# Anttwo/SuGaR

Hardware: AMD Instinct MI355X
Metric: train_step_images_per_sec (higher is better)
Workload: dtype f32; 1 GPU; metric: 1000000 Gaussians @ 1920x1080, SH degree 3, 3DGS train step (raster fwd -> 0.8 L1 + 0.2 DSSIM -> bwd -> Adam, 59 floats/Gaussian), 8 orbit cameras cycled; parallelism=view-sharded dp1, single process, no collective

## Files before the change

### include/sugar_raster.h

```cpp
#ifndef SUGAR_RASTER_H_INCLUDED
#define SUGAR_RASTER_H_INCLUDED

#include <stddef.h>
#include <stdint.h>

#ifdef __cplusplus
extern "C" {
#endif

#define SGR_ABI_VERSION 4

#define SGR_E_INVALID (-1)
#define SGR_E_HIP (-2)
#define SGR_E_ALLOC (-3)

typedef char* (*sgr_alloc_fn)(void* user, size_t bytes);

int sgr_abi_version(void);
const char* sgr_last_error(void);

int64_t sgr_forward(sgr_alloc_fn geom_alloc, void* geom_user,
                    sgr_alloc_fn binning_alloc, void* binning_user,
                    sgr_alloc_fn img_alloc, void* img_user,
                    int P, int D, int M,
// ... 78 lines not shown
                       char* geom_buffer, char* binning_buffer, char* img_buffer,
                       const float* dL_dpix,
                       float* dL_dmean2D, float* dL_dconic, float* dL_dopacity, float* dL_dcolor,
                       float* dL_dmean3D, float* dL_dcov3D, float* dL_dsh, float* dL_dscale, float* dL_drot,
                       int debug, void* stream);

typedef struct sgr_backward_opts {
    float* max_radii2D;
    float* grad_accum;
    float* denom;
    float* campos_row;
    int flags;
} sgr_backward_opts;
#define SGR_BWD_EXACT_ALPHA 2
#define SGR_BWD_TILE_ORDER_READY 1
int sgr_backward_ex(int phase, int P, int D, int M, int64_t R,
                    const float* background, int width, int height,
                    const float* means3D, const float* shs, const float* colors_precomp,
                    const float* scales, float scale_modifier, const float* rotations,
                    const float* cov3D_precomp, const float* viewmatrix, const float* projmatrix,
                    const float* cam_pos, float tan_fovx, float tan_fovy, const int* radii,
                    char* geom_buffer, char* binning_buffer, char* img_buffer,
                    const float* dL_dpix,
                    float* dL_dmean2D, float* dL_dconic, float* dL_dopacity, float* dL_dcolor,
                    float* dL_dmean3D, float* dL_dcov3D, float* dL_dsh, float* dL_dscale, float* dL_drot,
                    int debug, void* stream, const sgr_backward_opts* opts);

int sgr_sh_grad_from_views(int P, int n_views, int D, int M, const float* means3D, const float* campos_all,
                           const float* dcolor_all, int64_t view_stride, float* dL_dsh, void* stream);

// ... 3 lines not shown
                           float lr_rest, float beta1, float beta2, float eps, int step, float grad_scale, void* stream);

int sgr_sh_adam_from_views_ex(int P, int n_views, int D, int M, const float* means3D, const float* campos_all,
                              const float* dcolor_all, int64_t view_stride, float* sh_params, float* exp_avg, float* exp_avg_sq,
                              float lr_dc, float lr_rest, float beta1, float beta2, float eps, int step, float grad_scale,
                              float* dmean_extra, void* stream);

int sgr_mark_visible(int P, const float* means3D, const float* viewmatrix, const float* projmatrix,
                     uint8_t* present, void* stream);

size_t sgr_geom_bytes(int P);
size_t sgr_img_bytes(int width, int height);
size_t sgr_binning_bytes(int64_t R, int width, int height);

size_t sgr_geom_rec_offset(int P);
size_t sgr_img_final_T_offset(int width, int height);
size_t sgr_img_n_contrib_offset(int width, int height);
size_t sgr_img_tile_start_offset(int width, int height);
size_t sgr_img_tile_maxc_offset(int width, int height);
size_t sgr_img_tile_walked_offset(int width, int height);
size_t sgr_img_header_offset(int width, int height);
size_t sgr_binning_point_list_offset(int64_t R);

#define SGR_N_STAGES 15
void sgr_profile_enable(int stage_mask);
int sgr_profile_read(double* ms_sum, int64_t* count, int n_stages);


int sgr_dist2(int P, const float* points, float* meanDists, void* stream);
int sgr_knn(int N, const float* query, int M, const float* ref, int K, float* dists, int64_t* idx, void* stream);
// ... 62 lines not shown
    int64_t view_stride;
    const float* all_campos;
    float grad_scale;
    int step;
    int64_t g_begin, g_end;
    int64_t f_begin, f_end;
} sgr_train_exchange;
typedef struct sgr_trainer sgr_trainer;
sgr_trainer* sgr_trainer_create(const sgr_train_config* cfg);
void sgr_trainer_destroy(sgr_trainer* t);
int sgr_trainer_set_binning(sgr_trainer* t, char* binning, size_t bytes, int64_t capacity);
int sgr_trainer_step(sgr_trainer* t, const sgr_train_view* view, int phases, const sgr_train_exchange* ex, void* stream);
int sgr_trainer_set_exchange_chunks(sgr_trainer* t, int n);
int sgr_trainer_forward_valid(sgr_trainer* t, uint32_t* header_out);
const char* sgr_trainer_last_error(void);
int sgr_rccl_unique_id(char* out128);
int sgr_trainer_comm_init(sgr_trainer* t, const char* id128, int world, int rank, float* recv, size_t recv_bytes);
int sgr_trainer_comm_destroy(sgr_trainer* t);
int sgr_trainer_comm_abort(sgr_trainer* t);
int sgr_trainer_step_exchange(sgr_trainer* t, const sgr_train_view* view, int step, void* stream);
double sgr_trainer_last_exchange_wait_ms(sgr_trainer* t);
size_t sgr_bin2_bytes(int P, int width, int height);

int sgr_scaled_rotation_forward(int P, const float* quaternions, const float* scaling, int inverse_scales, float* out,
                                void* stream);
int sgr_scaled_rotation_backward(int P, const float* quaternions, const float* scaling, int inverse_scales,
                                 const float* dL_dout, float* dL_dquaternions, float* dL_dscaling, void* stream);

int sgr_pack_gaussians(int P, const float* centers, const float* inv_scaled_rot, const float* strengths, float* packed,
                       void* stream);
// ... 119 lines not shown
```

### sugar_amd/_lib.py

```python
from __future__ import annotations

import ctypes as C
import os

_HERE = os.path.dirname(os.path.abspath(__file__))
LIB_PATH = os.environ.get("SGR_LIB_PATH") or os.path.join(_HERE, "libsugar_raster.so")

ALLOC_FN = C.CFUNCTYPE(C.c_void_p, C.c_void_p, C.c_size_t)

_vp, _i, _f, _i64, _sz = C.c_void_p, C.c_int, C.c_float, C.c_int64, C.c_size_t
SIGNATURES = {
    "sgr_abi_version": (_i, []),
    "sgr_last_error": (C.c_char_p, []),
    "sgr_set_deep_min": (None, [_i]),
    "sgr_get_deep_min": (_i, []),
    "sgr_set_exact_alpha": (None, [_i]),
    "sgr_get_exact_alpha": (_i, []),
    "sgr_forward": (_i64, [ALLOC_FN, _vp, ALLOC_FN, _vp, ALLOC_FN, _vp, _i, _i, _i, _vp, _i, _i, _vp, _vp, _vp, _vp,
                           _vp, _f, _vp, _vp, _vp, _vp, _vp, _f, _f, _i, _vp, _vp, _i, _vp]),
    "sgr_forward_ex": (_i64, [ALLOC_FN, _vp, ALLOC_FN, _vp, ALLOC_FN, _vp, _i, _i, _i, _vp, _i, _i, _vp, _vp, _vp, _vp,
                              _vp, _f, _vp, _vp, _vp, _vp, _vp, _f, _f, _i, _vp, _vp, _i, _vp, _vp]),
    "sgr_backward": (_i, [_i, _i, _i, _i64, _vp, _i, _i, _vp, _vp, _vp, _vp, _f, _vp, _vp, _vp, _vp, _vp, _f, _f, _vp,
                          _vp, _vp, _vp, _vp, _vp, _vp, _vp, _vp, _vp, _vp, _vp, _vp, _vp, _i, _vp]),
    "sgr_backward_phase": (_i, [_i, _i, _i, _i, _i64, _vp, _i, _i, _vp, _vp, _vp, _vp, _f, _vp, _vp, _vp, _vp, _vp, _f, _f, _vp,
                                _vp, _vp, _vp, _vp, _vp, _vp, _vp, _vp, _vp, _vp, _vp, _vp, _vp, _i, _vp]),
    "sgr_backward_ex": (_i, [_i, _i, _i, _i, _i64, _vp, _i, _i, _vp, _vp, _vp, _vp, _f, _vp, _vp, _vp, _vp, _vp, _f, _f, _vp,
                             _vp, _vp, _vp, _vp, _vp, _vp, _vp, _vp, _vp, _vp, _vp, _vp, _vp, _i, _vp, _vp]),
    "sgr_mark_visible": (_i, [_i, _vp, _vp, _vp, _vp, _vp]),
    "sgr_trainer_create": (_vp, [_vp]),
    "sgr_trainer_destroy": (None, [_vp]),
    "sgr_trainer_set_binning": (_i, [_vp, _vp, _sz, _i64]),
    "sgr_trainer_step": (_i, [_vp, _vp, _i, _vp, _vp]),
    "sgr_trainer_forward_valid": (_i, [_vp, _vp]),
    "sgr_trainer_last_error": (C.c_char_p, []),
    "sgr_rccl_unique_id": (_i, [_vp]),
    "sgr_trainer_comm_init": (_i, [_vp, _vp, _i, _i, _vp, _sz]),
    "sgr_trainer_comm_destroy": (_i, [_vp]),
    "sgr_trainer_comm_abort": (_i, [_vp]),
    "sgr_trainer_step_exchange": (_i, [_vp, _vp, _i, _vp]),
    "sgr_trainer_set_exchange_chunks": (_i, [_vp, _i]),
    "sgr_trainer_last_exchange_wait_ms": (C.c_double, [_vp]),
    "sgr_bin2_bytes": (_sz, [_i, _i, _i]),
    "sgr_sh_grad_from_views": (_i, [_i, _i, _i, _i, _vp, _vp, _vp, _i64, _vp, _vp]),
    "sgr_sh_adam_from_views": (_i, [_i, _i, _i, _i, _vp, _vp, _vp, _i64, _vp, _vp, _vp, _f, _f, _f, _f, _f, _i, _f, _vp]),
    "sgr_sh_adam_from_views_ex": (_i, [_i, _i, _i, _i, _vp, _vp, _vp, _i64, _vp, _vp, _vp, _f, _f, _f, _f, _f, _i, _f, _vp, _vp]),
    "sgr_geom_bytes": (_sz, [_i]),
    "sgr_img_bytes": (_sz, [_i, _i]),
    "sgr_binning_bytes": (_sz, [_i64, _i, _i]),
    "sgr_geom_rec_offset": (_sz, [_i]),
    "sgr_img_final_T_offset": (_sz, [_i, _i]),
    "sgr_img_n_contrib_offset": (_sz, [_i, _i]),
    "sgr_img_tile_start_offset": (_sz, [_i, _i]),
    "sgr_img_tile_maxc_offset": (_sz, [_i, _i]),
    "sgr_img_tile_walked_offset": (_sz, [_i, _i]),
    "sgr_img_header_offset": (_sz, [_i, _i]),
    "sgr_binning_point_list_offset": (_sz, [_i64]),
    "sgr_profile_enable": (None, [_i]),
    "sgr_profile_read": (_i, [_vp, _vp, _i]),
    "sgr_l1_ssim_scratch_bytes": (_sz, [_i, _i, _i]),
    "sgr_l1_ssim_forward": (_i, [_i, _i, _i, _vp, _vp, _f, _vp, _vp, _vp]),
    "sgr_l1_ssim_backward": (_i, [_i, _i, _i, _vp, _vp, _f, _vp, _vp, _vp, _vp]),
    "sgr_l1_ssim_backward_ex": (_i, [_i, _i, _i, _vp, _vp, _f, _vp, _vp, _vp, _vp, _vp]),
    "sgr_adam_step": (_i, [C.c_longlong, _vp, _vp, _vp, _vp, _i, _vp, _vp, _vp, _vp, _vp, _vp, _f, _f, _f, _i, _f, _vp]),
    "sgr_adam_step_multi": (_i, [_i, _vp, _vp, _vp, _vp, _vp, _vp, _vp, _vp, _vp, _vp, _vp]),
# ... 84 lines not shown
                ("max_radii2D", _vp), ("grad_accum", _vp), ("denom", _vp)]


class TrainView(C.Structure):
    _fields_ = [("viewmatrix", _vp), ("projmatrix", _vp), ("campos", _vp), ("tan_fovx", _f), ("tan_fovy", _f), ("gt_image", _vp),
                ("tile_need", _vp), ("tile_need_out", _vp), ("hint_margin", _f), ("chunk_grid", C.c_uint32),
                ("tile_order", _vp), ("tile_order_out", _vp), ("flags", C.c_uint32)]


class TrainExchange(C.Structure):
    _fields_ = [("n_views", _i), ("all_colors", _vp), ("view_stride", _i64), ("all_campos", _vp), ("grad_scale", _f), ("step", _i),
                ("g_begin", _i64), ("g_end", _i64), ("f_begin", _i64), ("f_end", _i64)]


SGR_FLAG_RAW_PARAMS, SGR_FLAG_SINGLE_LEVEL_BINNING, SGR_FLAG_SPECULATIVE = 1, 2, 8
SGR_BWD_TILE_ORDER_READY = 1
HDR_R, HDR_HINT_MISS, HDR_L1_OVERFLOW = 0, 3, 6

_lib = None


def load() -> C.CDLL:
    global _lib
    if _lib is not None:
        return _lib
    if not os.path.exists(LIB_PATH):
        raise ImportError(
            f"{LIB_PATH} not found: the gfx950 HIP rasterizer is not built. Run `python -m sugar_amd.build` "
            "(or __graft_entry__.build()). There is no CPU fallback.")
    lib = C.CDLL(LIB_PATH)
    for name, (res, args) in SIGNATURES.items():
# ... 15 lines not shown
```

### sugar_amd/csrc/capi.hip

```cpp
#include "../../include/sugar_raster.h"
#include "sgr_common.h"
#include "tile_order.h"

#include <cstdlib>
#include <mutex>
#include <string>
#include <vector>

namespace {

thread_local std::string g_err;

int fail(int code, const std::string& msg)
{
    g_err = msg;
    return code;
}

#define HIP_TRY(expr)                                                                                   \
    do {                                                                                                \
        hipError_t e_ = (expr);                                                                         \
        if (e_ != hipSuccess)                                                                           \
            return fail(SGR_E_HIP, std::string(#expr) + ": " + hipGetErrorString(e_));                  \
    } while (0)
// ... 92 lines not shown

extern "C" {

int sgr_abi_version(void) { return SGR_ABI_VERSION; }
void sgr_set_deep_min(int entries) { g_deep_min = entries > 0 ? entries : 0; }
int sgr_get_deep_min(void) { return (int)sgr_deep_min(); }
void sgr_set_exact_alpha(int on) { g_exact_alpha = on ? 1 : 0; }
int sgr_get_exact_alpha(void) { return sgr_exact_alpha(); }

const char* sgr_last_error(void) { return g_err.c_str(); }

size_t sgr_geom_bytes(int P) { return sgr_geom_total(P); }
size_t sgr_img_bytes(int width, int height) { return sgr_img_layout(width, height).total; }
size_t sgr_binning_bytes(int64_t R, int width, int height) { return sgr_bin_layout(R, sgr_img_layout(width, height).T).total; }
size_t sgr_geom_rec_offset(int) { return 0; }
size_t sgr_img_final_T_offset(int w, int h) { return sgr_img_layout(w, h).final_T; }
size_t sgr_img_n_contrib_offset(int w, int h) { return sgr_img_layout(w, h).n_contrib; }
size_t sgr_img_tile_start_offset(int w, int h) { return sgr_img_layout(w, h).tile_start; }
size_t sgr_img_tile_maxc_offset(int w, int h) { return sgr_img_layout(w, h).tile_maxc; }
size_t sgr_img_tile_walked_offset(int w, int h) { return sgr_img_layout(w, h).tile_walked; }
size_t sgr_img_header_offset(int w, int h) { return sgr_img_layout(w, h).header; }
size_t sgr_binning_point_list_offset(int64_t R) { return sgr_bin_layout(R, 0).point_list; }

void sgr_profile_enable(int stage_mask) { g_prof.mask = (unsigned)stage_mask; }

int sgr_profile_read(double* ms_sum, int64_t* count, int n_stages)
{
    std::lock_guard<std::mutex> lk(g_prof_mu);
    for (int i = 0; i < n_stages; i++) { ms_sum[i] = 0.0; count[i] = 0; }
    for (auto& r : g_prof.recs) {
// ... 284 lines not shown
    job->T = IL.T;
    job->list_cap = (uint32_t)(R > 0xFFFFFFFFll ? 0xFFFFFFFFll : R);
    job->tile_maxc = reinterpret_cast<const uint32_t*>(img_buffer + IL.tile_maxc);
    job->tile_walked = opts->tile_need_out ? reinterpret_cast<const uint32_t*>(img_buffer + IL.tile_walked) : nullptr;
    job->header = reinterpret_cast<const uint32_t*>(img_buffer + IL.header);
    job->order = reinterpret_cast<uint32_t*>(img_buffer + IL.tile_cursor);
    job->order_copy = opts->tile_order_out;
    job->need_out = opts->tile_need_out;
    job->header_host = hh_dev;
    job->margin = opts->hint_margin > 0.f ? opts->hint_margin : 0.25f;
    job->gx = IL.gx;
    job->gy = IL.gy;
    return 0;
}

static int backward_impl(int phase, int P, int D, int M, int64_t R, const float* background, int width, int height,
                         const float* means3D, const float* shs, const float* colors_precomp, const float* scales,
                         float scale_modifier, const float* rotations, const float* cov3D_precomp, const float* viewmatrix,
                         const float* projmatrix, const float* cam_pos, float tan_fovx, float tan_fovy, char* geom_buffer,
                         char* binning_buffer, char* img_buffer, const float* dL_dpix, float* dL_dmean2D, float* dL_dconic,
                         float* dL_dopacity, float* dL_dcolor, float* dL_dmean3D, float* dL_dcov3D, float* dL_dsh,
                         float* dL_dscale, float* dL_drot, int debug, void* stream, const sgr_backward_opts* opts = nullptr)
{
    hipStream_t s = (hipStream_t)stream;
    const int raw_params = (phase & SGR_MODE_RAW_PARAMS) ? 1 : 0;
    const int sh_dir_elsewhere = (phase & SGR_MODE_SH_DIR_ELSEWHERE) ? 1 : 0;
    phase &= 3;
    if (phase < 0 || phase > 2) return fail(SGR_E_INVALID, "phase must be 0, 1 or 2");
    if (P <= 0 || width <= 0 || height <= 0) return fail(SGR_E_INVALID, "P, width and height must be positive");
    if (!geom_buffer || !binning_buffer || !img_buffer || !dL_dpix) return fail(SGR_E_INVALID, "null scratch / dL_dpix");
    if (!dL_dopacity || !dL_dcolor || !dL_dmean3D) return fail(SGR_E_INVALID, "null gradient output");
    if (cov3D_precomp && !dL_dcov3D) return fail(SGR_E_INVALID, "dL_dcov3D required with cov3D_precomp");
    const bool use_sh = shs && !colors_precomp;
    const bool compact = use_sh && !dL_dsh;
    if (!cov3D_precomp && (!dL_dscale || !dL_drot)) return fail(SGR_E_INVALID, "dL_dscale/dL_drot required");
    if (phase != 0 && !compact) return fail(SGR_E_INVALID, "the two-phase backward is for the compact SH mode");

    const ImgLayout IL = sgr_img_layout(width, height);
    const BinLayout BL = sgr_bin_layout(R, IL.T);
    const GeomRec* rec = reinterpret_cast<const GeomRec*>(geom_buffer);
    const float* final_T = reinterpret_cast<const float*>(img_buffer + IL.final_T);
    const uint32_t* n_contrib = reinterpret_cast<const uint32_t*>(img_buffer + IL.n_contrib);
    const uint32_t* tile_start = reinterpret_cast<const uint32_t*>(img_buffer + IL.tile_start);
    const uint32_t* blk_nb = reinterpret_cast<const uint32_t*>(img_buffer + IL.blk_nb);
    const uint32_t* point_list = reinterpret_cast<const uint32_t*>(binning_buffer + BL.point_list);

    float* acc = reinterpret_cast<float*>(geom_buffer + sgr_geom_acc_offset(P));
    if (phase != 2) {
        { SgrStageTimer t(s, SGR_STAGE_FILL); HIP_TRY(hipMemsetAsync(acc, 0, (size_t)P * SGR_ACC_STRIDE * 4, s)); }
        if (R > 0) {
            SgrStageTimer t(s, SGR_STAGE_BLEND_BWD);
            sgr_launch_blend_bwd(width, height, IL.gx, IL.gy, tile_start, point_list, binning_buffer, blk_nb, rec, background, final_T,
                                 n_contrib, dL_dpix, acc, reinterpret_cast<const uint32_t*>(img_buffer + IL.tile_maxc),
                                 reinterpret_cast<const uint32_t*>(img_buffer + IL.header), (uint32_t)(R > 0xFFFFFFFFll ? 0xFFFFFFFFll : R),
                                 reinterpret_cast<uint32_t*>(img_buffer + IL.tile_cursor),
                                 (opts && (opts->flags & SGR_BWD_TILE_ORDER_READY)) ? 1 : 0, s,
                                 (sgr_exact_alpha() || (opts && (opts->flags & SGR_BWD_EXACT_ALPHA))) ? 1 : 0);
        }
        STAGE_CHECK("blend_bwd");
        if (phase == 1) {
            { SgrStageTimer t(s, SGR_STAGE_MASKED_COLORS); sgr_launch_masked_colors(P, rec, acc, dL_dcolor, cam_pos, opts ? opts->campos_row : nullptr, s); }
            STAGE_CHECK("masked_colors");
            return 0;
        }
    }
    PreprocessBwdArgs pb;
    pb.P = P; pb.D = D; pb.M = use_sh ? M : 0;
    pb.means3D = means3D; pb.shs = use_sh ? shs : nullptr;
    pb.scales = cov3D_precomp ? nullptr : scales; pb.rotations = cov3D_precomp ? nullptr : rotations;
    pb.scale_modifier = scale_modifier; pb.cov3D_precomp = cov3D_precomp;
    pb.viewmatrix = viewmatrix; pb.projmatrix = projmatrix; pb.cam_pos = cam_pos;
    pb.W = width; pb.H = height; pb.tan_fovx = tan_fovx; pb.tan_fovy = tan_fovy;
    pb.focal_y = height / (2.0f * tan_fovy);
    pb.focal_x = width / (2.0f * tan_fovx);
    pb.rec = rec;
    pb.raw_params = raw_params && !cov3D_precomp;
    pb.sh_dir_elsewhere = sh_dir_elsewhere && use_sh && !dL_dsh;
    pb.acc = acc;
    pb.header = reinterpret_cast<const uint32_t*>(img_buffer + IL.header);
    pb.list_cap = (uint32_t)(R > 0xFFFFFFFFll ? 0xFFFFFFFFll : R);
    pb.campos_row = (opts && compact && phase == 0) ? opts->campos_row : nullptr;
    pb.dens_max_radii = opts ? opts->max_radii2D : nullptr;
    pb.dens_accum = opts ? opts->grad_accum : nullptr;
    pb.dens_denom = opts ? opts->denom : nullptr;
    pb.dL_dmean2D = dL_dmean2D; pb.dL_dconic = dL_dconic; pb.dL_dopacity = dL_dopacity;
    pb.dL_dcolor = phase == 2 ? nullptr : dL_dcolor;
    pb.dL_dmean3D = dL_dmean3D; pb.dL_dcov3D = dL_dcov3D; pb.dL_dsh = use_sh ? dL_dsh : nullptr;
    pb.dL_dscale = cov3D_precomp ? nullptr : dL_dscale; pb.dL_drot = cov3D_precomp ? nullptr : dL_drot;
    { SgrStageTimer t(s, SGR_STAGE_PREPROCESS_BWD); sgr_launch_preprocess_bwd(pb, s); }
    STAGE_CHECK("preprocess_bwd");
    return 0;
}

// ... 104 lines not shown
```

### sugar_amd/csrc/preprocess.hip

```cpp
#include "../../include/sugar_raster.h"
#include "sgr_common.h"

namespace {

__device__ __constant__ const float SH_C0 = 0.28209479177387814f;
__device__ __constant__ const float SH_C1 = 0.4886025119029199f;
__device__ __constant__ const float SH_C2[5] = {1.0925484305920792f, -1.0925484305920792f, 0.31539156525252005f,
                                                 -1.0925484305920792f, 0.5462742152960396f};
__device__ __constant__ const float SH_C3[7] = {-0.5900435899266435f, 2.890611442640554f, -0.4570457994644658f,
                                                 0.3731763325901154f, -0.4570457994644658f, 1.445305721320277f,
                                                 -0.5900435899266435f};

__device__ __forceinline__ float fmin_(float a, float b) { return a < b ? a : b; }
__device__ __forceinline__ float fmax_(float a, float b) { return a > b ? a : b; }

__device__ __forceinline__ int f2i_sat(float v)
{
    if (v != v) return 0;
    if (v >= 2147483648.0f) return 2147483647;
    if (v <= -2147483648.0f) return (-2147483647 - 1);
    return (int)v;
}

__device__ __forceinline__ float ndc2pix(float v, int S)
// ... 381 lines not shown
    uint32_t kmin = key, kmax = key == 0xFFFFFFFFu ? 0u : key;
    for (int o = 32; o > 0; o >>= 1) {
        kmin = min(kmin, (uint32_t)__shfl_xor((int)kmin, o));
        kmax = max(kmax, (uint32_t)__shfl_xor((int)kmax, o));
    }
    if ((threadIdx.x & 63) == 0) { s_mm[0][threadIdx.x >> 6] = kmin; s_mm[1][threadIdx.x >> 6] = kmax; }
    __syncthreads();
    if (threadIdx.x == 0)
        a.key_minmax[blockIdx.x] = make_uint2(min(min(s_mm[0][0], s_mm[0][1]), min(s_mm[0][2], s_mm[0][3])),
                                              max(max(s_mm[1][0], s_mm[1][1]), max(s_mm[1][2], s_mm[1][3])));
}

#ifndef SGR_PRE_BWD_BLOCKS
#define SGR_PRE_BWD_BLOCKS 3
#endif
template <bool STORE_SH, int SH>
__device__ __forceinline__ void preprocess_bwd_lane(const PreprocessBwdArgs& a, float* __restrict__ stage)
{
    const int idx0 = blockIdx.x * 256 + threadIdx.x;
    if (a.campos_row && idx0 < 3) a.campos_row[idx0] = a.cam_pos[idx0];
    uint32_t hdr_r = 0u, hdr_miss = 0u, hdr_ovf = 0u;
    if (a.header) { hdr_r = a.header[SGR_HDR_R]; hdr_miss = a.header[SGR_HDR_HINT_MISS]; hdr_ovf = a.header[4 + SGR_B2_HDR_OVERFLOW]; }
    const bool valid = idx0 < a.P;
    const int idx = valid ? idx0 : a.P - 1;
    const size_t i3 = 3 * (size_t)idx;
    const float cam_raw = cam_request(a.viewmatrix, a.projmatrix, a.cam_pos);
    const float4* rp4 = reinterpret_cast<const float4*>(a.rec + idx);
    const float4 rec0 = rp4[0], rec1 = rp4[1], rec2 = rp4[2];
    const float4* ap = reinterpret_cast<const float4*>(a.acc + SGR_ACC_STRIDE * (size_t)idx);
    const float4 s0 = ap[0], s1 = ap[1];
    const float s2x = a.acc[SGR_ACC_STRIDE * (size_t)idx + 8];
    const V3 mean = {a.means3D[i3], a.means3D[i3 + 1], a.means3D[i3 + 2]};
    float sc[3] = {0, 0, 0}, q[4] = {0, 0, 0, 0};
    float4 q_raw = make_float4(0.f, 0.f, 0.f, 0.f);
    float c6[6];
    if (a.cov3D_precomp) {
#pragma unroll
        for (int k = 0; k < 6; k++) c6[k] = a.cov3D_precomp[6 * (size_t)idx + k];
    } else {
        sc[0] = a.scales[i3]; sc[1] = a.scales[i3 + 1]; sc[2] = a.scales[i3 + 2];
        q_raw = *reinterpret_cast<const float4*>(a.rotations + 4 * (size_t)idx);
    }
    const int radius = __float_as_int(rec1.w);
    const uint32_t clamped = __float_as_uint(rec2.w);
    Cam cam;
    cam_unpack(cam_raw, cam);
    if (!valid) return;
    const bool fwd_invalid = hdr_r > a.list_cap || hdr_miss != 0u || hdr_ovf != 0u;
    const float* v = cam.vm;

    float dmean[3] = {0, 0, 0}, dcov[6] = {0, 0, 0, 0, 0, 0};
    const int n_sh = a.M * 3;
    if (fwd_invalid || !(radius > 0)) {
        if (a.dL_dmean2D) { a.dL_dmean2D[i3] = 0; a.dL_dmean2D[i3 + 1] = 0; a.dL_dmean2D[i3 + 2] = 0; }
        if (a.dL_dconic) { float4 z4 = {0, 0, 0, 0}; *reinterpret_cast<float4*>(a.dL_dconic + 4 * (size_t)idx) = z4; }
        a.dL_dopacity[idx] = 0;
        if (a.dL_dcolor) { a.dL_dcolor[i3] = 0; a.dL_dcolor[i3 + 1] = 0; a.dL_dcolor[i3 + 2] = 0; }
        a.dL_dmean3D[i3] = 0; a.dL_dmean3D[i3 + 1] = 0; a.dL_dmean3D[i3 + 2] = 0;
        if (a.dL_dcov3D) for (int k = 0; k < 6; k++) a.dL_dcov3D[6 * (size_t)idx + k] = 0;
        if (STORE_SH) {
            if (stage) {
#pragma unroll
                for (int k = 0; k < 48; k++) stage[65 * k] = 0.0f;
            } else {
                for (int k = 0; k < n_sh; k++) a.dL_dsh[(size_t)idx * n_sh + k] = 0;
            }
        }
        if (a.dL_dscale) { a.dL_dscale[i3] = 0; a.dL_dscale[i3 + 1] = 0; a.dL_dscale[i3 + 2] = 0; }
        if (a.dL_drot) { float4 z = {0, 0, 0, 0}; *reinterpret_cast<float4*>(a.dL_drot + 4 * (size_t)idx) = z; }
        return;
    }
    float sh[48];
    if (SH != 2) load_sh<48, SH == 0>(a.shs, idx, a.M, sh);
    if (!a.cov3D_precomp) {
        float4 q4 = q_raw;
        if (a.raw_params) {
            sc[0] = expf(sc[0]); sc[1] = expf(sc[1]); sc[2] = expf(sc[2]);
            const float inv = 1.0f / fmaxf(quat_norm_contracted(q4), 1e-12f);
            q4 = make_float4(q4.x * inv, q4.y * inv, q4.z * inv, q4.w * inv);
        }
        q[0] = q4.x; q[1] = q4.y; q[2] = q4.z; q[3] = q4.w;
        cov3d_from_scale_rot(sc, a.scale_modifier, q, c6);
    }
    float dcol[3], dm2x, dm2y;
    float g0, g1, g3;
    {
// ... 178 lines not shown
                                 __builtin_fmaf(-nz, dot, dq.z) * inv, __builtin_fmaf(-nw, dot, dq.w) * inv);
            } else {
                dq = make_float4(dq.x * 1e12f, dq.y * 1e12f, dq.z * 1e12f, dq.w * 1e12f);
            }
        }
        *reinterpret_cast<float4*>(a.dL_drot + 4 * (size_t)idx) = dq;
    }
    a.dL_dmean3D[i3] = dmean[0]; a.dL_dmean3D[i3 + 1] = dmean[1]; a.dL_dmean3D[i3 + 2] = dmean[2];
    if (a.dL_dcov3D) {
#pragma unroll
        for (int k = 0; k < 6; k++) a.dL_dcov3D[6 * (size_t)idx + k] = dcov[k];
    }
}

template <bool STORE_SH, int SH>
__global__ void __launch_bounds__(256, SGR_PRE_BWD_BLOCKS) k_preprocess_bwd(PreprocessBwdArgs a)
{
    __shared__ float s_stage[STORE_SH ? 4 * 48 * 65 : 1];
    const bool staged = STORE_SH && a.M == 16 && (((uintptr_t)a.dL_dsh) & 15) == 0;
    const int lane = threadIdx.x & 63, wave = threadIdx.x >> 6;
    float* panel = s_stage + (STORE_SH ? wave * (48 * 65) : 0);
    preprocess_bwd_lane<STORE_SH, SH>(a, staged ? panel + lane : nullptr);
    if (STORE_SH && staged) {
        __builtin_amdgcn_fence(__ATOMIC_ACQ_REL, "wavefront");
        __builtin_amdgcn_wave_barrier();
        const long long row0 = (long long)blockIdx.x * 256 + wave * 64;
        const int rows = (int)min(64ll, (long long)a.P - row0);
        float4* out4 = reinterpret_cast<float4*>(a.dL_dsh + (size_t)(row0 > 0 ? row0 : 0) * 48);
#pragma unroll
        for (int it = 0; it < 12; it++) {
            const int j4 = it * 64 + lane;
            if (j4 < rows * 12) {
                const int row = j4 / 12, e0 = (j4 % 12) * 4;
                const float* src = panel + 65 * e0 + row;
                out4[j4] = make_float4(src[0], src[65], src[130], src[195]);
            }
        }
// ... 412 lines not shown
```

### sugar_amd/csrc/sgr_common.h

```cpp
#pragma once
#include <cmath>
#include <cstdio>
#include <cstdlib>
#include <hip/hip_runtime.h>
#include <stdint.h>
#include <stddef.h>
#include "../../include/sugar_raster.h"

#define SGR_TILE_X 16
#define SGR_TILE_Y 16
#define SGR_TILE_PIX 256
#define SGR_NUM_CUS 256
#define SGR_LEGACY_LDS_BYTES (150 * 1024)
#define SGR_BIN_SLICES 1024

struct GeomRec {
    float x, y, cx, cy;
    float cz, opacity, depth;
    int radius;
    float r, g, b;
    uint32_t clamped;
};
static_assert(sizeof(GeomRec) == 48, "GeomRec must be 48 bytes");

static inline size_t sgr_align(size_t x, size_t a = 256) { return (x + a - 1) / a * a; }
static inline size_t sgr_geom_acc_offset(int P) { return sgr_align((size_t)(P > 0 ? P : 1) * 48); }
size_t sgr_sort_scratch_bytes(int P);
#define SGR_ACC_STRIDE 16
static inline size_t sgr_geom_sort_offset(int P) { return sgr_geom_acc_offset(P) + sgr_align((size_t)(P > 0 ? P : 1) * SGR_ACC_STRIDE * 4); }
size_t sgr_sort_rects_offset(int P);
static inline size_t sgr_geom_total(int P) { return sgr_geom_sort_offset(P) + sgr_sort_scratch_bytes(P); }

struct ImgLayout {
    size_t final_T, n_contrib, tile_start, tile_cursor, tile_maxc, tile_walked, blk_nb, header, repair_flag, repair_list, deep_list, blk_hist, total;
    int n_blocks;
    int gx, gy, T;
};
static inline ImgLayout sgr_img_layout(int W, int H)
{
    ImgLayout L;
    L.gx = (W + SGR_TILE_X - 1) / SGR_TILE_X;
    L.gy = (H + SGR_TILE_Y - 1) / SGR_TILE_Y;
    L.T = L.gx * L.gy;
    size_t off = 0;
    L.final_T = off;     off = sgr_align(off + (size_t)W * H * 4);
// ... 76 lines not shown
void sgr_launch_mark_visible(int P, const float* means3D, const float* viewmatrix, uint8_t* present, hipStream_t s);
void sgr_launch_preprocess_fwd(const PreprocessArgs& a, hipStream_t s);
void sgr_launch_depth_keys(const PreprocessArgs& a, hipStream_t s);

struct PreprocessBwdArgs {
    int P, D, M;
    const float* means3D; const float* shs; const float* scales; const float* rotations; float scale_modifier;
    const float* cov3D_precomp; const float* viewmatrix; const float* projmatrix; const float* cam_pos;
    int W, H; float tan_fovx, tan_fovy, focal_x, focal_y;
    const GeomRec* rec;
    int raw_params;
    int sh_dir_elsewhere;
    float* campos_row;
    float* dens_max_radii; float* dens_accum; float* dens_denom;
    const uint32_t* header; uint32_t list_cap;
    const float* acc;
    float* dL_dmean2D; float* dL_dconic; float* dL_dopacity; float* dL_dcolor;
    float* dL_dmean3D; float* dL_dcov3D; float* dL_dsh; float* dL_dscale; float* dL_drot;
};
void sgr_launch_preprocess_bwd(const PreprocessBwdArgs& a, hipStream_t s);
void sgr_launch_masked_colors(int P, const GeomRec* rec, const float* acc, float* out, const float* cam_pos, float* campos_row, hipStream_t s);
void sgr_launch_sh_grad_from_views(int P, int V, int D, int M, size_t vstride, const float* means3D, const float* campos,
                                   const float* dcolor, float* dL_dsh, hipStream_t s);

static inline double sgr_intended_double(float x)
{
    static thread_local float memo_x[2] = {0.f, 0.f};
    static thread_local double memo_d[2] = {0.0, 0.0};
    for (int k = 0; k < 2; k++) if (memo_x[k] == x && memo_x[k] != 0.f) return memo_d[k];
    double out = (double)x;
    char buf[48];
// ... 72 lines not shown
```

### sugar_amd/csrc/train.hip

```cpp
#include "../../include/sugar_raster.h"
#include "sgr_common.h"
#include "tile_order.h"

#include <chrono>
#include <cmath>
#include <cstdlib>
#include <cstring>
#include <dlfcn.h>
#include <string>

namespace {

struct FixedBuf { char* p; size_t bytes; size_t asked; };
char* fixed_alloc(void* user, size_t bytes)
{
    FixedBuf* b = static_cast<FixedBuf*>(user);
    b->asked = bytes;
    return bytes <= b->bytes ? b->p : nullptr;
}

struct RcclUniqueId { char internal[128]; };
typedef void* RcclComm;
struct Rccl {
    void* handle = nullptr;
// ... 34 lines not shown
}

struct sgr_trainer {
    sgr_train_config c;
    RcclComm comm = nullptr;
    int world = 1, rank = 0;
    hipStream_t comm_stream = nullptr;
    hipEvent_t ev_colors = nullptr, ev_small = nullptr;
    int chunks = 1;
    hipEvent_t ev_gathered[16] = {}, ev_reduced[16] = {};
    float* recv = nullptr;
    float* campos_all = nullptr;
    double last_wait_ms = 0.0;
    hipEvent_t hdr_event = nullptr;
    bool have_forward = false;
    bool defer_post = false;
    int64_t R = 0;
    long long seg_begin[4], seg_end[4];
    float seg_lr[4];
    int seg_one[4];
    std::string err;
};

extern "C" {

static thread_local std::string g_train_err;
static int tfail(int code, const std::string& m) { g_train_err = m; return code; }
const char* sgr_trainer_last_error(void) { return g_train_err.c_str(); }

sgr_trainer* sgr_trainer_create(const sgr_train_config* cfg)
// ... 30 lines not shown
void sgr_trainer_destroy(sgr_trainer* t)
{
    if (!t) return;
    (void)sgr_trainer_comm_destroy(t);
    if (t->hdr_event) (void)hipEventDestroy(t->hdr_event);
    delete t;
}

int sgr_trainer_set_binning(sgr_trainer* t, char* binning, size_t bytes, int64_t capacity)
{
    if (!t || !binning || capacity <= 0 || bytes < sgr_binning_bytes(capacity, t->c.width, t->c.height))
        return tfail(SGR_E_INVALID, "sgr_trainer_set_binning: bad buffer");
    t->c.binning = binning; t->c.binning_bytes = bytes; t->c.binning_capacity = capacity;
    return 0;
}

int sgr_trainer_forward_valid(sgr_trainer* t, uint32_t* header_out)
{
    if (!t || !t->have_forward) return tfail(SGR_E_INVALID, "sgr_trainer_forward_valid: no forward yet");
    if (hipEventSynchronize(t->hdr_event) != hipSuccess) return tfail(SGR_E_HIP, "hipEventSynchronize failed");
    const uint32_t* h = t->c.header_host;
    if (header_out) std::memcpy(header_out, h, 64);
    const bool bad = (int64_t)h[SGR_HDR_R] > t->R || h[8 + SGR_HDR_HINT_MISS] != 0u || h[SGR_HDR_L1_OVERFLOW] != 0u;
    return bad ? 0 : 1;
}

int sgr_trainer_step(sgr_trainer* t, const sgr_train_view* v, int phases, const sgr_train_exchange* ex, void* stream)
{
    if (!t || !v) return tfail(SGR_E_INVALID, "sgr_trainer_step: null argument");
    const sgr_train_config& c = t->c;
// ... 30 lines not shown
        if (R < 0) return tfail((int)R, std::string("forward: ") + sgr_last_error());
        t->R = R;
        t->have_forward = true;
        SgrTileOrderJob job = {};
        int rc = t->defer_post ? sgr_forward_post_job(W, H, c.img, R, &fo, &job) : 0;
        if (rc < 0) return tfail(rc, "sgr_forward_post_job failed");
        { SgrStageTimer tm(s, SGR_STAGE_LOSS_FWD); rc = sgr_l1_ssim_forward_job(3, W, H, c.image, v->gt_image, c.lambda_dssim, c.loss_scratch, nullptr, t->defer_post ? &job : nullptr, stream); }
        if (rc < 0) return tfail(rc, "l1_ssim_forward failed");
        if (t->defer_post && hipEventRecord(t->hdr_event, s) != hipSuccess) return tfail(SGR_E_HIP, "hipEventRecord failed");
        { SgrStageTimer tm(s, SGR_STAGE_LOSS_BWD); rc = sgr_l1_ssim_backward_ex(3, W, H, c.image, v->gt_image, c.lambda_dssim, c.loss_scratch, nullptr, c.grad_image, c.loss_out, stream); }
        if (rc < 0) return tfail(rc, "l1_ssim_backward failed");
    }
    if (phases & 3) {
        if (!t->have_forward) return tfail(SGR_E_INVALID, "sgr_trainer_step: backward before any forward");
        sgr_backward_opts bo = {c.max_radii2D, c.grad_accum, c.denom, c.colors + 3 * (size_t)P,
                                (t->defer_post || v->tile_order_out) ? SGR_BWD_TILE_ORDER_READY : 0};
        const int first = (phases & 3) == 3 ? 0 : ((phases & 1) ? 1 : 2);
        const int last = (phases & 3) == 3 ? 0 : ((phases & 2) ? 2 : 1);
        for (int ph = first; ph <= last; ph++) {
            const int rc = sgr_backward_ex(ph | SGR_MODE_RAW_PARAMS, P, c.D, c.M, t->R, c.background, W, H, means3D, shs, nullptr, scal,
                                           1.0f, rot, nullptr, v->viewmatrix, v->projmatrix, v->campos, v->tan_fovx, v->tan_fovy,
                                           c.radii, c.geom, c.binning, c.img, c.grad_image, c.dL_dmean2D, nullptr,
                                           grad + c.off_opacity, c.colors, grad + c.off_xyz, nullptr, nullptr, grad + c.off_scaling,
                                           grad + c.off_rotation, 0, stream, &bo);
            if (rc < 0) return tfail(rc, std::string("backward: ") + sgr_last_error());
        }
    }
    if (phases & 12) {
        if (!ex || ex->step < 1 || ex->n_views < 1) return tfail(SGR_E_INVALID, "sgr_trainer_step: exchange description missing");
        float bc1, bc2_sqrt;
        sgr_bias_corrections(c.beta1, c.beta2, ex->step, &bc1, &bc2_sqrt);
        if (phases & 4) {
            const float* cols = ex->all_colors ? ex->all_colors : c.colors;
            const float* cams = ex->all_campos ? ex->all_campos : (ex->all_colors ? nullptr : c.colors + 3 * (size_t)P);
            if (!cams) return tfail(SGR_E_INVALID, "sgr_trainer_step: all_campos missing");
            const size_t stride = (size_t)(ex->view_stride ? ex->view_stride : (ex->all_colors ? P : P + 1));
            const bool part = ex->g_end > ex->g_begin;
            const long long g0 = part ? ex->g_begin : 0, g1 = part ? ex->g_end : P;
            if (g0 < 0 || g1 > P || (g0 & 63)) return tfail(SGR_E_INVALID, "sgr_trainer_step: bad Gaussian range (g_begin must be a multiple of 64)");
            if (part && !ex->all_colors) cols += 3 * (size_t)g0;
// ... 172 lines not shown
```

Measured before the change: 981.3 images/s.

## Skip accumulator memset and untouched-Gaussian backward work via in-kernel cleanup

The preprocess backward kernel now zeroes the per-Gaussian blend accumulator rows it reads, so the trainer can skip the full accumulator memset before each backward. When a wave has many dirty rows it clears a contiguous block; otherwise each dirty lane clears its own row. Gaussians whose accumulator is all zero (never touched by blending) now take the zero-gradient path instead of the full chain-rule computation, unless a dense flag is set. This removes a large memset and redundant math for invisible-in-practice Gaussians, at the cost of extra writes in the kernel and reliance on state tracking across steps.

```diff
diff --git a/include/sugar_raster.h b/include/sugar_raster.h
--- a/include/sugar_raster.h
+++ b/include/sugar_raster.h
@@ -116,6 +116,8 @@
 } sgr_backward_opts;
 #define SGR_BWD_EXACT_ALPHA 2
 #define SGR_BWD_TILE_ORDER_READY 1
+#define SGR_BWD_DENSE 8
+#define SGR_BWD_ACC_CLEAN 4
 int sgr_backward_ex(int phase, int P, int D, int M, int64_t R,
                     const float* background, int width, int height,
                     const float* means3D, const float* shs, const float* colors_precomp,
@@ -149,6 +151,7 @@
 size_t sgr_binning_bytes(int64_t R, int width, int height);
 
 size_t sgr_geom_rec_offset(int P);
+size_t sgr_geom_acc_offset_bytes(int P);
 size_t sgr_img_final_T_offset(int width, int height);
 size_t sgr_img_n_contrib_offset(int width, int height);
 size_t sgr_img_tile_start_offset(int width, int height);
@@ -241,6 +244,7 @@
 int sgr_trainer_set_exchange_chunks(sgr_trainer* t, int n);
 int sgr_trainer_forward_valid(sgr_trainer* t, uint32_t* header_out);
 const char* sgr_trainer_last_error(void);
+int sgr_trainer_acc_dirty(sgr_trainer* t);
 int sgr_rccl_unique_id(char* out128);
 int sgr_trainer_comm_init(sgr_trainer* t, const char* id128, int world, int rank, float* recv, size_t recv_bytes);
 int sgr_trainer_comm_destroy(sgr_trainer* t);
diff --git a/sugar_amd/_lib.py b/sugar_amd/_lib.py
--- a/sugar_amd/_lib.py
+++ b/sugar_amd/_lib.py
@@ -33,6 +33,7 @@
     "sgr_trainer_step": (_i, [_vp, _vp, _i, _vp, _vp]),
     "sgr_trainer_forward_valid": (_i, [_vp, _vp]),
     "sgr_trainer_last_error": (C.c_char_p, []),
+    "sgr_trainer_acc_dirty": (_i, [_vp]),
     "sgr_rccl_unique_id": (_i, [_vp]),
     "sgr_trainer_comm_init": (_i, [_vp, _vp, _i, _i, _vp, _sz]),
     "sgr_trainer_comm_destroy": (_i, [_vp]),
@@ -48,6 +49,7 @@
     "sgr_img_bytes": (_sz, [_i, _i]),
     "sgr_binning_bytes": (_sz, [_i64, _i, _i]),
     "sgr_geom_rec_offset": (_sz, [_i]),
+    "sgr_geom_acc_offset_bytes": (_sz, [_i]),
     "sgr_img_final_T_offset": (_sz, [_i, _i]),
     "sgr_img_n_contrib_offset": (_sz, [_i, _i]),
     "sgr_img_tile_start_offset": (_sz, [_i, _i]),
@@ -162,7 +164,7 @@
 
 
 SGR_FLAG_RAW_PARAMS, SGR_FLAG_SINGLE_LEVEL_BINNING, SGR_FLAG_SPECULATIVE = 1, 2, 8
-SGR_BWD_TILE_ORDER_READY = 1
+SGR_BWD_TILE_ORDER_READY, SGR_BWD_ACC_CLEAN, SGR_BWD_DENSE = 1, 4, 8
 HDR_R, HDR_HINT_MISS, HDR_L1_OVERFLOW = 0, 3, 6
 
 _lib = None
diff --git a/sugar_amd/csrc/capi.hip b/sugar_amd/csrc/capi.hip
--- a/sugar_amd/csrc/capi.hip
+++ b/sugar_amd/csrc/capi.hip
@@ -130,6 +130,7 @@
 size_t sgr_img_bytes(int width, int height) { return sgr_img_layout(width, height).total; }
 size_t sgr_binning_bytes(int64_t R, int width, int height) { return sgr_bin_layout(R, sgr_img_layout(width, height).T).total; }
 size_t sgr_geom_rec_offset(int) { return 0; }
+size_t sgr_geom_acc_offset_bytes(int P) { return sgr_geom_acc_offset(P); }
 size_t sgr_img_final_T_offset(int w, int h) { return sgr_img_layout(w, h).final_T; }
 size_t sgr_img_n_contrib_offset(int w, int h) { return sgr_img_layout(w, h).n_contrib; }
 size_t sgr_img_tile_start_offset(int w, int h) { return sgr_img_layout(w, h).tile_start; }
@@ -444,6 +445,14 @@
     return 0;
 }
 
+}
+hipError_t sgr_acc_reset(char* geom_buffer, int P, hipStream_t s)
+{
+    SgrStageTimer t(s, SGR_STAGE_FILL);
+    return hipMemsetAsync(geom_buffer + sgr_geom_acc_offset(P), 0, (size_t)P * SGR_ACC_STRIDE * 4, s);
+}
+extern "C" {
+
 static int backward_impl(int phase, int P, int D, int M, int64_t R, const float* background, int width, int height,
                          const float* means3D, const float* shs, const float* colors_precomp, const float* scales,
                          float scale_modifier, const float* rotations, const float* cov3D_precomp, const float* viewmatrix,
@@ -464,7 +473,7 @@
     const bool use_sh = shs && !colors_precomp;
     const bool compact = use_sh && !dL_dsh;
     if (!cov3D_precomp && (!dL_dscale || !dL_drot)) return fail(SGR_E_INVALID, "dL_dscale/dL_drot required");
-    if (phase != 0 && !compact) return fail(SGR_E_INVALID, "the two-phase backward is for the compact SH mode");
+    if (phase == 1 && !compact) return fail(SGR_E_INVALID, "the two-phase backward is for the compact SH mode");
 
     const ImgLayout IL = sgr_img_layout(width, height);
     const BinLayout BL = sgr_bin_layout(R, IL.T);
@@ -476,8 +485,9 @@
     const uint32_t* point_list = reinterpret_cast<const uint32_t*>(binning_buffer + BL.point_list);
 
     float* acc = reinterpret_cast<float*>(geom_buffer + sgr_geom_acc_offset(P));
+    const bool acc_clean = opts && (opts->flags & SGR_BWD_ACC_CLEAN);
     if (phase != 2) {
-        { SgrStageTimer t(s, SGR_STAGE_FILL); HIP_TRY(hipMemsetAsync(acc, 0, (size_t)P * SGR_ACC_STRIDE * 4, s)); }
+        if (!acc_clean) HIP_TRY(sgr_acc_reset(geom_buffer, P, s));
         if (R > 0) {
             SgrStageTimer t(s, SGR_STAGE_BLEND_BWD);
             sgr_launch_blend_bwd(width, height, IL.gx, IL.gy, tile_start, point_list, binning_buffer, blk_nb, rec, background, final_T,
@@ -507,6 +517,8 @@
     pb.raw_params = raw_params && !cov3D_precomp;
     pb.sh_dir_elsewhere = sh_dir_elsewhere && use_sh && !dL_dsh;
     pb.acc = acc;
+    pb.acc_clean = acc_clean ? 1 : 0;
+    pb.dense = (opts && (opts->flags & SGR_BWD_DENSE)) ? 1 : 0;
     pb.header = reinterpret_cast<const uint32_t*>(img_buffer + IL.header);
     pb.list_cap = (uint32_t)(R > 0xFFFFFFFFll ? 0xFFFFFFFFll : R);
     pb.campos_row = (opts && compact && phase == 0) ? opts->campos_row : nullptr;
diff --git a/sugar_amd/csrc/preprocess.hip b/sugar_amd/csrc/preprocess.hip
--- a/sugar_amd/csrc/preprocess.hip
+++ b/sugar_amd/csrc/preprocess.hip
@@ -419,22 +419,61 @@
 #ifndef SGR_PRE_BWD_BLOCKS
 #define SGR_PRE_BWD_BLOCKS 3
 #endif
+struct BwdHead { float4 rec0, rec1, rec2, s0, s1; float s2x; };
+__device__ __forceinline__ void bwd_head_load(const PreprocessBwdArgs& a, int idx, BwdHead& h)
+{
+    const float4* rp4 = reinterpret_cast<const float4*>(a.rec + idx);
+    h.rec0 = rp4[0]; h.rec1 = rp4[1]; h.rec2 = rp4[2];
+    const float4* ap = reinterpret_cast<const float4*>(a.acc + SGR_ACC_STRIDE * (size_t)idx);
+    h.s0 = ap[0]; h.s1 = ap[1];
+    h.s2x = a.acc[SGR_ACC_STRIDE * (size_t)idx + 8];
+}
+__device__ __forceinline__ bool bwd_touched(const float4 s0, const float4 s1, const float s2x)
+{
+    return !(s0.x == 0.f && s0.y == 0.f && s0.z == 0.f && s0.w == 0.f && s1.x == 0.f && s1.y == 0.f && s1.z == 0.f && s1.w == 0.f &&
+             s2x == 0.f);
+}
+__device__ __forceinline__ void bwd_acc_clean(const PreprocessBwdArgs& a, int idx)
+{
+    float4* ap = reinterpret_cast<float4*>(a.acc + SGR_ACC_STRIDE * (size_t)idx);
+    const float4 z4 = {0.f, 0.f, 0.f, 0.f};
+    ap[0] = z4; ap[1] = z4;
+    a.acc[SGR_ACC_STRIDE * (size_t)idx + 8] = 0.f;
+}
+template <bool STORE_SH>
+__device__ __forceinline__ void bwd_zero_row(const PreprocessBwdArgs& a, int idx, float* __restrict__ stage, bool stats, int radius)
+{
+    const size_t i3 = 3 * (size_t)idx;
+    const int n_sh = a.M * 3;
+    if (a.dL_dmean2D) { a.dL_dmean2D[i3] = 0; a.dL_dmean2D[i3 + 1] = 0; a.dL_dmean2D[i3 + 2] = 0; }
+    if (a.dL_dconic) { float4 z4 = {0, 0, 0, 0}; *reinterpret_cast<float4*>(a.dL_dconic + 4 * (size_t)idx) = z4; }
+    a.dL_dopacity[idx] = 0;
+    if (a.dL_dcolor) { a.dL_dcolor[i3] = 0; a.dL_dcolor[i3 + 1] = 0; a.dL_dcolor[i3 + 2] = 0; }
+    a.dL_dmean3D[i3] = 0; a.dL_dmean3D[i3 + 1] = 0; a.dL_dmean3D[i3 + 2] = 0;
+    if (a.dL_dcov3D) for (int k = 0; k < 6; k++) a.dL_dcov3D[6 * (size_t)idx + k] = 0;
+    if (STORE_SH) {
+        if (stage) {
+#pragma unroll
+            for (int k = 0; k < 48; k++) stage[65 * k] = 0.0f;
+        } else {
+            for (int k = 0; k < n_sh; k++) a.dL_dsh[(size_t)idx * n_sh + k] = 0;
+        }
+    }
+    if (a.dL_dscale) { a.dL_dscale[i3] = 0; a.dL_dscale[i3 + 1] = 0; a.dL_dscale[i3 + 2] = 0; }
+    if (a.dL_drot) { float4 z = {0, 0, 0, 0}; *reinterpret_cast<float4*>(a.dL_drot + 4 * (size_t)idx) = z; }
+    if (stats) {
+        if (a.dens_denom) a.dens_denom[idx] += 1.0f;
+        if (a.dens_max_radii) a.dens_max_radii[idx] = fmaxf(a.dens_max_radii[idx], (float)radius);
+    }
+}
+
 template <bool STORE_SH, int SH>
-__device__ __forceinline__ void preprocess_bwd_lane(const PreprocessBwdArgs& a, float* __restrict__ stage)
-{
-    const int idx0 = blockIdx.x * 256 + threadIdx.x;
-    if (a.campos_row && idx0 < 3) a.campos_row[idx0] = a.cam_pos[idx0];
-    uint32_t hdr_r = 0u, hdr_miss = 0u, hdr_ovf = 0u;
-    if (a.header) { hdr_r = a.header[SGR_HDR_R]; hdr_miss = a.header[SGR_HDR_HINT_MISS]; hdr_ovf = a.header[4 + SGR_B2_HDR_OVERFLOW]; }
-    const bool valid = idx0 < a.P;
-    const int idx = valid ? idx0 : a.P - 1;
+__device__ __forceinline__ void bwd_full_row(const PreprocessBwdArgs& a, const int idx, const BwdHead& h, const Cam& cam,
+                                             float* __restrict__ stage)
+{
     const size_t i3 = 3 * (size_t)idx;
-    const float cam_raw = cam_request(a.viewmatrix, a.projmatrix, a.cam_pos);
-    const float4* rp4 = reinterpret_cast<const float4*>(a.rec + idx);
-    const float4 rec0 = rp4[0], rec1 = rp4[1], rec2 = rp4[2];
-    const float4* ap = reinterpret_cast<const float4*>(a.acc + SGR_ACC_STRIDE * (size_t)idx);
-    const float4 s0 = ap[0], s1 = ap[1];
-    const float s2x = a.acc[SGR_ACC_STRIDE * (size_t)idx + 8];
+    const float4 rec0 = h.rec0, rec1 = h.rec1, rec2 = h.rec2, s0 = h.s0, s1 = h.s1;
+    const float s2x = h.s2x;
     const V3 mean = {a.means3D[i3], a.means3D[i3 + 1], a.means3D[i3 + 2]};
     float sc[3] = {0, 0, 0}, q[4] = {0, 0, 0, 0};
     float4 q_raw = make_float4(0.f, 0.f, 0.f, 0.f);
@@ -448,33 +487,9 @@
     }
     const int radius = __float_as_int(rec1.w);
     const uint32_t clamped = __float_as_uint(rec2.w);
-    Cam cam;
-    cam_unpack(cam_raw, cam);
-    if (!valid) return;
-    const bool fwd_invalid = hdr_r > a.list_cap || hdr_miss != 0u || hdr_ovf != 0u;
     const float* v = cam.vm;
-
     float dmean[3] = {0, 0, 0}, dcov[6] = {0, 0, 0, 0, 0, 0};
     const int n_sh = a.M * 3;
-    if (fwd_invalid || !(radius > 0)) {
-        if (a.dL_dmean2D) { a.dL_dmean2D[i3] = 0; a.dL_dmean2D[i3 + 1] = 0; a.dL_dmean2D[i3 + 2] = 0; }
-        if (a.dL_dconic) { float4 z4 = {0, 0, 0, 0}; *reinterpret_cast<float4*>(a.dL_dconic + 4 * (size_t)idx) = z4; }
-        a.dL_dopacity[idx] = 0;
-        if (a.dL_dcolor) { a.dL_dcolor[i3] = 0; a.dL_dcolor[i3 + 1] = 0; a.dL_dcolor[i3 + 2] = 0; }
-        a.dL_dmean3D[i3] = 0; a.dL_dmean3D[i3 + 1] = 0; a.dL_dmean3D[i3 + 2] = 0;
-        if (a.dL_dcov3D) for (int k = 0; k < 6; k++) a.dL_dcov3D[6 * (size_t)idx + k] = 0;
-        if (STORE_SH) {
-            if (stage) {
-#pragma unroll
-                for (int k = 0; k < 48; k++) stage[65 * k] = 0.0f;
-            } else {
-                for (int k = 0; k < n_sh; k++) a.dL_dsh[(size_t)idx * n_sh + k] = 0;
-            }
-        }
-        if (a.dL_dscale) { a.dL_dscale[i3] = 0; a.dL_dscale[i3 + 1] = 0; a.dL_dscale[i3 + 2] = 0; }
-        if (a.dL_drot) { float4 z = {0, 0, 0, 0}; *reinterpret_cast<float4*>(a.dL_drot + 4 * (size_t)idx) = z; }
-        return;
-    }
     float sh[48];
     if (SH != 2) load_sh<48, SH == 0>(a.shs, idx, a.M, sh);
     if (!a.cov3D_precomp) {
@@ -683,13 +698,55 @@
 }
 
 template <bool STORE_SH, int SH>
+__device__ __forceinline__ void preprocess_bwd_lane(const PreprocessBwdArgs& a, float* __restrict__ stage, const int idx0)
+{
+    if (a.campos_row && idx0 < 3) a.campos_row[idx0] = a.cam_pos[idx0];
+    uint32_t hdr_r = 0u, hdr_miss = 0u, hdr_ovf = 0u;
+    if (a.header) { hdr_r = a.header[SGR_HDR_R]; hdr_miss = a.header[SGR_HDR_HINT_MISS]; hdr_ovf = a.header[4 + SGR_B2_HDR_OVERFLOW]; }
+    const bool valid = idx0 < a.P;
+    const int idx = valid ? idx0 : a.P - 1;
+    const float cam_raw = cam_request(a.viewmatrix, a.projmatrix, a.cam_pos);
+    BwdHead h;
+    bwd_head_load(a, idx, h);
+    Cam cam;
+    cam_unpack(cam_raw, cam);
+    if (a.acc_clean) {
+        const bool dirty = valid && bwd_touched(h.s0, h.s1, h.s2x);
+        const unsigned long long m = __ballot(dirty);
+        if (__popcll(m) >= 32) {
+            const int lane = threadIdx.x & 63;
+            const long long row0 = (long long)idx0 - lane;
+            float4* w4 = reinterpret_cast<float4*>(a.acc + SGR_ACC_STRIDE * (size_t)row0);
+            const float4 z4 = {0.f, 0.f, 0.f, 0.f};
+#pragma unroll
+            for (int i = 0; i < 4; i++) {
+                const int j = i * 64 + lane;
+                if (row0 + (j >> 2) < (long long)a.P) w4[j] = z4;
+            }
+        } else if (dirty) {
+            bwd_acc_clean(a, idx);
+        }
+    }
+    if (!valid) return;
+    const bool fwd_invalid = hdr_r > a.list_cap || hdr_miss != 0u || hdr_ovf != 0u;
+    const int radius = __float_as_int(h.rec1.w);
+    const bool touched = bwd_touched(h.s0, h.s1, h.s2x);
+    const bool rendered = !fwd_invalid && radius > 0;
+    if (!rendered || !(touched || a.dense)) {
+        bwd_zero_row<STORE_SH>(a, idx, stage, rendered, radius);
+        return;
+    }
+    bwd_full_row<STORE_SH, SH>(a, idx, h, cam, stage);
+}
+
+template <bool STORE_SH, int SH>
 __global__ void __launch_bounds__(256, SGR_PRE_BWD_BLOCKS) k_preprocess_bwd(PreprocessBwdArgs a)
 {
     __shared__ float s_stage[STORE_SH ? 4 * 48 * 65 : 1];
     const bool staged = STORE_SH && a.M == 16 && (((uintptr_t)a.dL_dsh) & 15) == 0;
     const int lane = threadIdx.x & 63, wave = threadIdx.x >> 6;
     float* panel = s_stage + (STORE_SH ? wave * (48 * 65) : 0);
-    preprocess_bwd_lane<STORE_SH, SH>(a, staged ? panel + lane : nullptr);
+    preprocess_bwd_lane<STORE_SH, SH>(a, staged ? panel + lane : nullptr, blockIdx.x * 256 + threadIdx.x);
     if (STORE_SH && staged) {
         __builtin_amdgcn_fence(__ATOMIC_ACQ_REL, "wavefront");
         __builtin_amdgcn_wave_barrier();
diff --git a/sugar_amd/csrc/sgr_common.h b/sugar_amd/csrc/sgr_common.h
--- a/sugar_amd/csrc/sgr_common.h
+++ b/sugar_amd/csrc/sgr_common.h
@@ -29,6 +29,7 @@
 #define SGR_ACC_STRIDE 16
 static inline size_t sgr_geom_sort_offset(int P) { return sgr_geom_acc_offset(P) + sgr_align((size_t)(P > 0 ? P : 1) * SGR_ACC_STRIDE * 4); }
 size_t sgr_sort_rects_offset(int P);
+hipError_t sgr_acc_reset(char* geom_buffer, int P, hipStream_t s);
 static inline size_t sgr_geom_total(int P) { return sgr_geom_sort_offset(P) + sgr_sort_scratch_bytes(P); }
 
 struct ImgLayout {
@@ -135,7 +136,9 @@
     float* campos_row;
     float* dens_max_radii; float* dens_accum; float* dens_denom;
     const uint32_t* header; uint32_t list_cap;
-    const float* acc;
+    float* acc;
+    int acc_clean;
+    int dense;
     float* dL_dmean2D; float* dL_dconic; float* dL_dopacity; float* dL_dcolor;
     float* dL_dmean3D; float* dL_dcov3D; float* dL_dsh; float* dL_dscale; float* dL_drot;
 };
diff --git a/sugar_amd/csrc/train.hip b/sugar_amd/csrc/train.hip
--- a/sugar_amd/csrc/train.hip
+++ b/sugar_amd/csrc/train.hip
@@ -72,6 +72,7 @@
     double last_wait_ms = 0.0;
     hipEvent_t hdr_event = nullptr;
     bool have_forward = false;
+    bool acc_dirty = true;
     bool defer_post = false;
     int64_t R = 0;
     long long seg_begin[4], seg_end[4];
@@ -132,6 +133,8 @@
     t->c.binning = binning; t->c.binning_bytes = bytes; t->c.binning_capacity = capacity;
     return 0;
 }
+
+int sgr_trainer_acc_dirty(sgr_trainer* t) { return (t && !t->acc_dirty) ? 0 : 1; }
 
 int sgr_trainer_forward_valid(sgr_trainer* t, uint32_t* header_out)
 {
@@ -192,16 +195,22 @@
     if (phases & 3) {
         if (!t->have_forward) return tfail(SGR_E_INVALID, "sgr_trainer_step: backward before any forward");
         sgr_backward_opts bo = {c.max_radii2D, c.grad_accum, c.denom, c.colors + 3 * (size_t)P,
-                                (t->defer_post || v->tile_order_out) ? SGR_BWD_TILE_ORDER_READY : 0};
+                                ((t->defer_post || v->tile_order_out) ? SGR_BWD_TILE_ORDER_READY : 0) | SGR_BWD_ACC_CLEAN};
         const int first = (phases & 3) == 3 ? 0 : ((phases & 1) ? 1 : 2);
         const int last = (phases & 3) == 3 ? 0 : ((phases & 2) ? 2 : 1);
         for (int ph = first; ph <= last; ph++) {
+            if (ph != 2) {
+                if (t->acc_dirty && sgr_acc_reset(c.geom, P, s) != hipSuccess)
+                    return tfail(SGR_E_HIP, "sgr_trainer_step: accumulator reset failed");
+                t->acc_dirty = true;
+            }
             const int rc = sgr_backward_ex(ph | SGR_MODE_RAW_PARAMS, P, c.D, c.M, t->R, c.background, W, H, means3D, shs, nullptr, scal,
                                            1.0f, rot, nullptr, v->viewmatrix, v->projmatrix, v->campos, v->tan_fovx, v->tan_fovy,
                                            c.radii, c.geom, c.binning, c.img, c.grad_image, c.dL_dmean2D, nullptr,
                                            grad + c.off_opacity, c.colors, grad + c.off_xyz, nullptr, nullptr, grad + c.off_scaling,
                                            grad + c.off_rotation, 0, stream, &bo);
             if (rc < 0) return tfail(rc, std::string("backward: ") + sgr_last_error());
+            if (ph != 1) t->acc_dirty = false;
         }
     }
     if (phases & 12) {
```

Result: faster. 1017 images/s, median of 6 (+3.6%).
